# QuackenbushLab/phoenix

Hardware: AMD Instinct MI355X
Metric: ODE-RHS evals/sec (genes x trajectories) (higher is better)
Workload: dtype f32; 1 GPU; C4 breast_cancer ~11k-gene pseudotime, 256 trajectory intervals/GPU, dopri5 + adjoint; genes=11165, hidden=40, trajectories_per_gpu=256, method=dopri5, parallelism=trajectory-sharded x1, grouped gradient all-reduce, status_readback=deferred

## Files before the change

phoenix_amd/csrc/phx_adj3t.hip:

```cpp
#include <hip/hip_runtime.h>

#include <cstdlib>

#include "phx_solver.hpp"
#include "phx_host.hpp"

using namespace phxh;

#include "phx_mfma_common.inc"
#include "phx_mfma_v3common.inc"
#include "phx_mfma_adj3_tail.inc"

namespace phxh {

bool adj3_tail_on(const SolveArgs &a)
{
    const char *e = getenv("PHX_V3_TAIL");
    if (e && e[0] == '0') return false;
    const bool forced = e && e[0] == '1';
    return a.grads && a.d.HT == 3 && a.d.TG <= 256 && (forced || a.d.TG * a.d.ntg >= 4) &&
           (long long)tail_record_floats(a.d.Bt, a.d.ntg) <= a.PP;
}

bool launch_adj3_tail(const SolveArgs &a, const phx_grads *g, int overwrite, hipStream_t st)
{
    const D1 &d = a.d;
    hipLaunchKernelGGL((k3_tail_adj3<3>), dim3((unsigned int)(2 * d.nblk)), dim3(256), 0, st, d, a.w, a.net.g,
                       a.grad_y, a.adj_y0, a.PP, g->Ws, g->Wp, g->WaT, g->g, g->bs, g->bp, overwrite, g->Wa);
    return hipGetLastError() == hipSuccess;
}

}

extern "C" int phx_debug_adj3_tail_words(size_t *deferred, size_t *served)
{
    if (deferred) *deferred = (size_t)XH_DEFER * 4;
    if (served) *served = (size_t)XH_SERVED * 4;
    const char *e = getenv("PHX_V3_TAIL");
    return (e && e[0] == '0') ? 0 : 1;
}
```

phoenix_amd/csrc/phx_mfma_adj3_tail.inc:

```
namespace {

template <int HT>
__global__ __launch_bounds__(256, 2) void k3_tail_adj3(D1 d, W1 w, const float *__restrict__ gmul,
                                                       const float *__restrict__ grad_y, float *adj_y0, long long PP, float *gWs, float *gWp, float *gWaT,
                                                       float *gg, float *gbs, float *gbp, int overwrite, float *gWa)
{
    constexpr int F4 = 4 * HT, F2 = 2 * HT;
    __shared__ float4 red[4][F4][64];
    __shared__ __attribute__((aligned(16))) float ctl[4][16 * TR_N];
    __shared__ float dgred[4][16], bred[4][2][HT * 16];
    __shared__ int sdef[256];
    const int tid = threadIdx.x, lane = tid & 63, li = lane & 15, lq = lane >> 4;
    const int wv = __builtin_amdgcn_readfirstlane(tid >> 6);
    const int item = blockIdx.x, gb = item >> 1, s2 = item & 1;
    const int gtile = gb / d.NB, bl = gb % d.NB;
    const int N = d.N, H = d.H, B = d.B, Bt = d.Bt, ntg = d.ntg, TG = d.TG, G = d.G;
    const bool bias_item = item == 0;
    unsigned int *hdr = reinterpret_cast<unsigned int *>(w.cnt);
    for (int i = tid; i < 256; i += blockDim.x) sdef[i] = (i < TG && hdr[XH_DEFER + i] == 1u) ? 1 : 0;
    __syncthreads();

    const int tiles_wg = ntg * d.NB;
    const int lane32h = lane * 32 + 16 * s2, lane16 = lane * 16;
    const int gene0 = gb * 32;
    const long long og = (long long)d.nblk * (F4 * 2 * 256), obs = og + N, obp = obs + H;
    const __amdgpu_buffer_rsrc_t hrs = make_rsrc(w.hq, (unsigned int)((size_t)TG * ntg * 7 * F4 * 1024));
    auto ring = [&](int kb, int j) -> int { const int v = kb + j; return v >= 7 ? v - 7 : v; };
    float rr[4];
#pragma unroll
    for (int j = 0; j < 4; ++j) {
        const int gene = gene0 + gmap(lq, 4 * s2 + j);
        const float gm = gene < N ? gmul[gene] : 0.f;
        rr[j] = gm > 0.f ? gm : 0.f;
    }
    f32x4 gs_[HT], gp_[HT], ga_[F2];
    float dgacc[4], sbias[HT], pbias[HT];
#pragma unroll
    for (int f = 0; f < HT; ++f) { gs_[f] = (f32x4){0.f, 0.f, 0.f, 0.f}; gp_[f] = gs_[f]; sbias[f] = 0.f; pbias[f] = 0.f; }
#pragma unroll
    for (int f = 0; f < F2; ++f) ga_[f] = (f32x4){0.f, 0.f, 0.f, 0.f};
#pragma unroll
    for (int j = 0; j < 4; ++j) dgacc[j] = 0.f;

    for (int tt = wv; tt < TG * ntg; tt += 4) {
        const int grp = tt / ntg, ttl = tt % ntg;
        if (!sdef[grp]) continue;
        const float *blk = w.dtheta + (long long)grp * PP;
        __builtin_amdgcn_fence(__ATOMIC_SEQ_CST, "wavefront");
        reinterpret_cast<float4 *>(ctl[wv])[lane] = reinterpret_cast<const float4 *>(blk + (long long)ttl * 16 * TR_N)[lane];
        __builtin_amdgcn_fence(__ATOMIC_SEQ_CST, "wavefront");
        const int kb = __builtin_amdgcn_readfirstlane(reinterpret_cast<const int *>(blk + (long long)Bt * TR_N)[ttl]);
        const float *rec = ctl[wv] + li * TR_N;
        const int b = grp * Bt + ttl * 16 + li;
        const bool okb = b < B;
        const __amdgpu_buffer_rsrc_t trs = make_rsrc(w.scratch + (long long)(grp * G + gtile) * d.nvec * tiles_wg * 512,
                                                     (unsigned int)(d.nvec * tiles_wg * 2048));
        auto toff = [&](int v) -> int { return ((v * tiles_wg) + (ttl * d.NB + bl)) * 2048; };
        auto hoff = [&](int slot, int f) -> int { return (((grp * ntg + ttl) * 7 + slot) * F4 + f) * 1024; };
        float y0v[4], a0v[4], ky[7][4], ka[7][4];
        bload4(trs, lane32h, toff(C_Y0), y0v);
        bload4(trs, lane32h, toff(C_A0), a0v);
#pragma unroll
        for (int j = 0; j < 7; ++j) {
            bload4(trs, lane32h, toff(C_KY + ring(kb, j)), ky[j]);
            bload4(trs, lane32h, toff(C_KA + ring(kb, j)), ka[j]);
        }
        const float dts = rec[TR_DT], sg = rec[TR_SG];
        auto weighted = [&](int S) -> bool { return __any(rec[TR_W + S] != 0.f) != 0; };
        float h[F4][4];
        auto issue_h = [&](int S) {
            const int hs = ring(kb, S);
#pragma unroll
            for (int f = 0; f < F4; ++f) bload4(hrs, lane16, hoff(hs, (f + F2) % F4), h[f]);
        };
        if (weighted(0)) issue_h(0);
        float a1[4];
        auto stage = [&](auto Sc) {
            constexpr int S = decltype(Sc)::value;
            asm volatile("; PHXMARK tail stage %0" ::"n"(S));
            float ys[4], as[4];
            if (S == 0) {
#pragma unroll
                for (int j = 0; j < 4; ++j) { ys[j] = y0v[j]; as[j] = a0v[j]; }
            } else {
                float sy[4], sa[4];
#pragma unroll
                for (int j = 0; j < 4; ++j) { sy[j] = 0.f; sa[j] = 0.f; }
#pragma unroll
                for (int kk = 0; kk < S; ++kk) {
                    const float cf = DP_BETA[S > 0 ? S - 1 : 0][kk] * dts;
#pragma unroll
                    for (int j = 0; j < 4; ++j) { sy[j] += ky[kk][j] * cf; sa[j] += ka[kk][j] * cf; }
                }
#pragma unroll
                for (int j = 0; j < 4; ++j) { ys[j] = y0v[j] + sy[j]; as[j] = a0v[j] + sa[j]; }
            }
            if (S == 6) {
#pragma unroll
                for (int j = 0; j < 4; ++j) a1[j] = as[j];
            }
            if (weighted(S)) {
                const float wl = rec[TR_W + S];
                float w4[4];
#pragma unroll
                for (int r = 0; r < 4; ++r) w4[r] = ctl[wv][(4 * lq + r) * TR_N + TR_W + S];
                float an[4], ln[4], qn[4];
                act_pair_fast_pk<2>(ys, an, ln);
#pragma unroll
                for (int j = 0; j < 4; ++j) {
                    qn[j] = as[j] * rr[j];
                    dgacc[j] += wl * (as[j] * (-sg * ky[S][j]));
                }
                float at[4], lt[4], qt[4];
                xpose4(an, at, lane);
                xpose4(ln, lt, lane);
                xpose4(qn, qt, lane);
#pragma unroll
                for (int r = 0; r < 4; ++r) { at[r] *= w4[r]; lt[r] *= w4[r]; qt[r] *= w4[r]; }
#pragma unroll
                for (int f = 0; f < HT; ++f)
#pragma unroll
                    for (int r = 0; r < 4; ++r) {
                        gs_[f] = mfma4(h[f][r], at[r], gs_[f]);
                        gp_[f] = mfma4(h[HT + f][r], lt[r], gp_[f]);
                    }
#pragma unroll
                for (int f = 0; f < F2; ++f)
#pragma unroll
                    for (int r = 0; r < 4; ++r) ga_[f] = mfma4(h[F2 + f][r], qt[r], ga_[f]);
                if (bias_item) {
#pragma unroll
                    for (int f = 0; f < HT; ++f) {
                        sbias[f] += ((w4[0] * h[f][0] + w4[1] * h[f][1]) + w4[2] * h[f][2]) + w4[3] * h[f][3];
                        pbias[f] += ((w4[0] * h[HT + f][0] + w4[1] * h[HT + f][1]) + w4[2] * h[HT + f][2]) + w4[3] * h[HT + f][3];
                    }
                }
            }
            __builtin_amdgcn_sched_barrier(0);
            if (S < 6 && weighted(S < 6 ? S + 1 : 6)) issue_h(S + 1);
        };
        stage(I3<0>{}); stage(I3<1>{}); stage(I3<2>{}); stage(I3<3>{}); stage(I3<4>{}); stage(I3<5>{});
        const bool adv = rec[TR_ADV] != 0.f;
        float gy4[4];
        {
            const long long ro = (long long)b * N;
            const int g0 = gene0 + gmap(lq, 4 * s2);
            row_load4(grad_y, ro, g0, N, okb && adv, 0.f, gy4);
        }
        stage(I3<6>{});
        asm volatile("; PHXMARK tail accept");
        {
            float am[4];
#pragma unroll
            for (int j = 0; j < 4; ++j) am[j] = ka[0][j] * (dts * DP_CMID[0]);
#pragma unroll
            for (int kk = 2; kk < 6; ++kk) {
                const float cf = dts * DP_CMID[kk];
#pragma unroll
                for (int j = 0; j < 4; ++j) am[j] += ka[kk][j] * cf;
            }
            const InterpX ix = {rec[TR_X], rec[TR_X + 1], rec[TR_X + 2], rec[TR_X + 3]};
            float anew[4];
#pragma unroll
            for (int j = 0; j < 4; ++j) {
                am[j] += ka[6][j] * (dts * DP_CMID[6]);
                const float aout = interp_eval(a0v[j], a1[j], a0v[j] + am[j], ka[0][j], ka[6][j], dts, ix);
                anew[j] = adv ? aout + gy4[j] : a0v[j];
            }
            row_store4(adj_y0, (long long)b * N, gene0 + gmap(lq, 4 * s2), N, okb, anew);
        }
    }

#pragma unroll
    for (int f = 0; f < HT; ++f) {
        red[wv][0 * HT + f][lane] = make_float4(gs_[f][0], gs_[f][1], gs_[f][2], gs_[f][3]);
        red[wv][1 * HT + f][lane] = make_float4(gp_[f][0], gp_[f][1], gp_[f][2], gp_[f][3]);
        red[wv][2 * HT + f][lane] = make_float4(ga_[f][0], ga_[f][1], ga_[f][2], ga_[f][3]);
        red[wv][3 * HT + f][lane] = make_float4(ga_[HT + f][0], ga_[HT + f][1], ga_[HT + f][2], ga_[HT + f][3]);
    }
#pragma unroll
    for (int j = 0; j < 4; ++j) {
        float v = rr[j] > 0.f ? dgacc[j] * fast_rcp(rr[j]) : 0.f;
        v += __shfl_xor(v, 1, 64); v += __shfl_xor(v, 2, 64); v += __shfl_xor(v, 4, 64); v += __shfl_xor(v, 8, 64);
        if (li == 0) dgred[wv][lq * 4 + j] = v;
    }
    if (bias_item) {
#pragma unroll
        for (int f = 0; f < HT; ++f) {
            float sb = sbias[f], sp = pbias[f];
            sb += __shfl_xor(sb, 16, 64); sb += __shfl_xor(sb, 32, 64);
            sp += __shfl_xor(sp, 16, 64); sp += __shfl_xor(sp, 32, 64);
            if (lq == 0) { bred[wv][0][f * 16 + li] = sb; bred[wv][1][f * 16 + li] = sp; }
        }
    }
    __syncthreads();

    for (int mf = wv; mf < F4; mf += 4) {
        float4 sacc = red[0][mf][lane];
#pragma unroll
        for (int k = 1; k < 4; ++k) {
            const float4 v = red[k][mf][lane];
            sacc.x += v.x; sacc.y += v.y; sacc.z += v.z; sacc.w += v.w;
        }
        const long long slot = ((long long)gb * (F4 * 2) + mf * 2 + s2) * 64 + lane;
        for (int g = 0; g < TG; ++g)
            if (!sdef[g]) {
                const float4 v = reinterpret_cast<const float4 *>(w.dtheta + (long long)g * PP)[slot];
                sacc.x += v.x; sacc.y += v.y; sacc.z += v.z; sacc.w += v.w;
            }
        const int m = mf / HT, f = mf % HT;
        const int gene = gene0 + gmapC(li, s2);
        float *dst = (m == 0) ? gWs : (m == 1 ? gWp : (m == 2 ? gWaT : gWaT + (long long)H * N));
        const float o[4] = {sacc.x, sacc.y, sacc.z, sacc.w};
        if (gene >= N) continue;
        if (gWa && m >= 2) {
            float *q = gWa + (long long)gene * 2 * H + (m - 2) * H + 16 * f;
#pragma unroll
            for (int r = 0; r < 4; ++r) {
                const int rw = rho16(lq, r);
                if (16 * f + rw < H) q[rw] = overwrite ? o[r] : q[rw] + o[r];
            }
        } else {
#pragma unroll
            for (int r = 0; r < 4; ++r) {
                const int row = 16 * f + rho16(lq, r);
                if (row < H) {
                    float *q = dst + (long long)row * N + gene;
                    *q = overwrite ? o[r] : *q + o[r];
                }
            }
        }
    }
    if (tid < 16) {
        const int gene = gene0 + gmap(tid >> 2, 4 * s2 + (tid & 3));
        if (gene < N) {
            float v = ((dgred[0][tid] + dgred[1][tid]) + dgred[2][tid]) + dgred[3][tid];
            for (int g = 0; g < TG; ++g)
                if (!sdef[g]) v += w.dtheta[(long long)g * PP + og + gene];
            gg[gene] = overwrite ? v : gg[gene] + v;
        }
    }
    if (bias_item && tid >= 64 && tid < 64 + HT * 16) {
        const int e = tid - 64, f = e >> 4, i = e & 15;
        const int hid = 16 * f + rho16(i >> 2, i & 3);
        if (hid < H) {
            float sb = ((bred[0][0][e] + bred[1][0][e]) + bred[2][0][e]) + bred[3][0][e];
            float sp = ((bred[0][1][e] + bred[1][1][e]) + bred[2][1][e]) + bred[3][1][e];
            for (int g = 0; g < TG; ++g)
                if (!sdef[g]) { sb += w.dtheta[(long long)g * PP + obs + hid]; sp += w.dtheta[(long long)g * PP + obp + hid]; }
            gbs[hid] = overwrite ? sb : gbs[hid] + sb;
            gbp[hid] = overwrite ? sp : gbp[hid] + sp;
        }
    }
    if (bias_item && tid == 0) {
        int n = 0;
        for (int g = 0; g < TG; ++g) n += sdef[g];
        hdr[XH_SERVED] = (unsigned int)n;
    }
}

}
```

Baseline: 61.57 billion gene*trajectory RHS evals/s.

## Prefetch adjoint tail hidden rows into LDS across stages and tiles

Adds a default path (REGROWS=false) that streams the per-stage hidden-activation rows directly into LDS with buffer_load_lds and prefetches the next weighted stage, including the first weighted stage of the next served tile. Stage weight masks and ring offsets are peeked one tile ahead, and loads are interleaved with MFMAs through sched_group_barrier. It also makes FMA contraction explicit and moves the grad_y load into stage 5. The aim is to hide global-load latency of the h rows behind MFMA work, at the cost of hand-written waitcnt encodings and LDS reuse of the reduction buffer.

```diff
diff --git a/phoenix_amd/csrc/phx_adj3t.hip b/phoenix_amd/csrc/phx_adj3t.hip
--- a/phoenix_amd/csrc/phx_adj3t.hip
+++ b/phoenix_amd/csrc/phx_adj3t.hip
@@ -17,7 +17,7 @@
 {
     const char *e = getenv("PHX_V3_TAIL");
     if (e && e[0] == '0') return false;
-    const bool forced = e && e[0] == '1';
+    const bool forced = e && (e[0] == '1' || e[0] == '2');
     return a.grads && a.d.HT == 3 && a.d.TG <= 256 && (forced || a.d.TG * a.d.ntg >= 4) &&
            (long long)tail_record_floats(a.d.Bt, a.d.ntg) <= a.PP;
 }
@@ -25,7 +25,9 @@
 bool launch_adj3_tail(const SolveArgs &a, const phx_grads *g, int overwrite, hipStream_t st)
 {
     const D1 &d = a.d;
-    hipLaunchKernelGGL((k3_tail_adj3<3>), dim3((unsigned int)(2 * d.nblk)), dim3(256), 0, st, d, a.w, a.net.g,
+    const char *e = getenv("PHX_V3_TAIL");
+    auto kern = (e && e[0] == '2') ? k3_tail_adj3<3, true> : k3_tail_adj3<3, false>;
+    hipLaunchKernelGGL(kern, dim3((unsigned int)(2 * d.nblk)), dim3(256), 0, st, d, a.w, a.net.g,
                        a.grad_y, a.adj_y0, a.PP, g->Ws, g->Wp, g->WaT, g->g, g->bs, g->bp, overwrite, g->Wa);
     return hipGetLastError() == hipSuccess;
 }
diff --git a/phoenix_amd/csrc/phx_mfma_adj3_tail.inc b/phoenix_amd/csrc/phx_mfma_adj3_tail.inc
--- a/phoenix_amd/csrc/phx_mfma_adj3_tail.inc
+++ b/phoenix_amd/csrc/phx_mfma_adj3_tail.inc
@@ -1,10 +1,11 @@
 namespace {
 
-template <int HT>
+template <int HT, bool REGROWS>
 __global__ __launch_bounds__(256, 2) void k3_tail_adj3(D1 d, W1 w, const float *__restrict__ gmul,
                                                        const float *__restrict__ grad_y, float *adj_y0, long long PP, float *gWs, float *gWp, float *gWaT,
                                                        float *gg, float *gbs, float *gbp, int overwrite, float *gWa)
 {
+#pragma clang fp contract(off)
     constexpr int F4 = 4 * HT, F2 = 2 * HT;
     __shared__ float4 red[4][F4][64];
     __shared__ __attribute__((aligned(16))) float ctl[4][16 * TR_N];
@@ -42,21 +43,55 @@
 #pragma unroll
     for (int j = 0; j < 4; ++j) dgacc[j] = 0.f;
 
-    for (int tt = wv; tt < TG * ntg; tt += 4) {
+    const int T4 = TG * ntg;
+    auto next_served = [&](int tq) -> int {
+        do tq += 4; while (tq < T4 && __builtin_amdgcn_readfirstlane(sdef[tq / ntg]) == 0);
+        return tq;
+    };
+    auto peek_load = [&](int tq, float4 &wa, float4 &wb, int &kbq) {
+        const float *blk = w.dtheta + (long long)(tq / ntg) * PP;
+        const int tl = tq % ntg;
+        const float4 *r4 = reinterpret_cast<const float4 *>(blk + ((long long)tl * 16 + li) * TR_N + TR_W);
+        wa = r4[0]; wb = r4[1];
+        kbq = reinterpret_cast<const int *>(blk + (long long)Bt * TR_N)[tl];
+    };
+    auto peek_mask = [&](const float4 &wa, const float4 &wb) -> int {
+        const float ws[7] = {wa.x, wa.y, wa.z, wa.w, wb.x, wb.y, wb.z};
+        int m = 0;
+#pragma unroll
+        for (int S = 0; S < 7; ++S) m |= (__any(ws[S] != 0.f) != 0 ? 1 : 0) << S;
+        return __builtin_amdgcn_readfirstlane(m);
+    };
+    auto request = [&](int tq, int kbq, int S) {
+        const int base = ((tq * 7 + ring(kbq, S)) * F4) * 1024;
+#pragma unroll
+        for (int f = 0; f < F4; ++f)
+            __builtin_amdgcn_raw_ptr_buffer_load_lds(hrs, (__attribute__((address_space(3))) void *)&red[wv][f][0], 16,
+                                                     lane16, base + ((f + F2) % F4) * 1024, 0, 0);
+    };
+    int tt = next_served(wv - 4), kb = 0, mask = 0;
+    if (tt < T4) {
+        float4 wa, wb;
+        peek_load(tt, wa, wb, kb);
+        kb = __builtin_amdgcn_readfirstlane(kb);
+        mask = peek_mask(wa, wb);
+        if (!REGROWS && mask) request(tt, kb, __builtin_ctz(mask));
+    }
+    while (tt < T4) {
         const int grp = tt / ntg, ttl = tt % ntg;
-        if (!sdef[grp]) continue;
+        const int tn = next_served(tt);
+        float4 nwa, nwb;
+        int nkb;
+        peek_load(tn < T4 ? tn : tt, nwa, nwb, nkb);
         const float *blk = w.dtheta + (long long)grp * PP;
-        __builtin_amdgcn_fence(__ATOMIC_SEQ_CST, "wavefront");
-        reinterpret_cast<float4 *>(ctl[wv])[lane] = reinterpret_cast<const float4 *>(blk + (long long)ttl * 16 * TR_N)[lane];
-        __builtin_amdgcn_fence(__ATOMIC_SEQ_CST, "wavefront");
-        const int kb = __builtin_amdgcn_readfirstlane(reinterpret_cast<const int *>(blk + (long long)Bt * TR_N)[ttl]);
+        const float4 recs = reinterpret_cast<const float4 *>(blk + (long long)ttl * 16 * TR_N)[lane];
         const float *rec = ctl[wv] + li * TR_N;
         const int b = grp * Bt + ttl * 16 + li;
         const bool okb = b < B;
         const __amdgpu_buffer_rsrc_t trs = make_rsrc(w.scratch + (long long)(grp * G + gtile) * d.nvec * tiles_wg * 512,
                                                      (unsigned int)(d.nvec * tiles_wg * 2048));
         auto toff = [&](int v) -> int { return ((v * tiles_wg) + (ttl * d.NB + bl)) * 2048; };
-        auto hoff = [&](int slot, int f) -> int { return (((grp * ntg + ttl) * 7 + slot) * F4 + f) * 1024; };
+        auto hoff = [&](int slot, int f) -> int { return ((tt * 7 + slot) * F4 + f) * 1024; };
         float y0v[4], a0v[4], ky[7][4], ka[7][4];
         bload4(trs, lane32h, toff(C_Y0), y0v);
         bload4(trs, lane32h, toff(C_A0), a0v);
@@ -65,15 +100,23 @@
             bload4(trs, lane32h, toff(C_KY + ring(kb, j)), ky[j]);
             bload4(trs, lane32h, toff(C_KA + ring(kb, j)), ka[j]);
         }
+        __builtin_amdgcn_fence(__ATOMIC_SEQ_CST, "wavefront");
+        reinterpret_cast<float4 *>(ctl[wv])[lane] = recs;
+        __builtin_amdgcn_fence(__ATOMIC_SEQ_CST, "wavefront");
         const float dts = rec[TR_DT], sg = rec[TR_SG];
-        auto weighted = [&](int S) -> bool { return __any(rec[TR_W + S] != 0.f) != 0; };
+        const bool adv = rec[TR_ADV] != 0.f;
+        nkb = __builtin_amdgcn_readfirstlane(nkb);
+        const int nmask = tn < T4 ? peek_mask(nwa, nwb) : 0;
+        auto weighted = [&](int S) -> bool { return ((mask >> S) & 1) != 0; };
+        if (!REGROWS && mask == 0 && nmask) request(tn, nkb, __builtin_ctz(nmask));
         float h[F4][4];
         auto issue_h = [&](int S) {
             const int hs = ring(kb, S);
 #pragma unroll
             for (int f = 0; f < F4; ++f) bload4(hrs, lane16, hoff(hs, (f + F2) % F4), h[f]);
         };
-        if (weighted(0)) issue_h(0);
+        if (REGROWS && weighted(0)) issue_h(0);
+        float gy4[4];
         float a1[4];
         auto stage = [&](auto Sc) {
             constexpr int S = decltype(Sc)::value;
@@ -90,7 +133,7 @@
                 for (int kk = 0; kk < S; ++kk) {
                     const float cf = DP_BETA[S > 0 ? S - 1 : 0][kk] * dts;
 #pragma unroll
-                    for (int j = 0; j < 4; ++j) { sy[j] += ky[kk][j] * cf; sa[j] += ka[kk][j] * cf; }
+                    for (int j = 0; j < 4; ++j) { sy[j] = __builtin_fmaf(ky[kk][j], cf, sy[j]); sa[j] = __builtin_fmaf(ka[kk][j], cf, sa[j]); }
                 }
 #pragma unroll
                 for (int j = 0; j < 4; ++j) { ys[j] = y0v[j] + sy[j]; as[j] = a0v[j] + sa[j]; }
@@ -99,17 +142,42 @@
 #pragma unroll
                 for (int j = 0; j < 4; ++j) a1[j] = as[j];
             }
+            auto load_gy = [&]() {
+                const long long ro = (long long)b * N;
+                const int g0 = gene0 + gmap(lq, 4 * s2);
+                row_load4(grad_y, ro, g0, N, okb && adv, 0.f, gy4);
+            };
             if (weighted(S)) {
                 const float wl = rec[TR_W + S];
                 float w4[4];
+                int rbase = 0;
 #pragma unroll
                 for (int r = 0; r < 4; ++r) w4[r] = ctl[wv][(4 * lq + r) * TR_N + TR_W + S];
+                if (!REGROWS) {
+                    asm volatile("" ::: "memory");
+                    __builtin_amdgcn_s_waitcnt(0x0F70);
+                    asm volatile("" ::: "memory");
+#pragma unroll
+                    for (int f = 0; f < F4; ++f) {
+                        const float4 v = red[wv][f][lane];
+                        h[f][0] = v.x; h[f][1] = v.y; h[f][2] = v.z; h[f][3] = v.w;
+                    }
+                    asm volatile("" ::: "memory");
+                    __builtin_amdgcn_s_waitcnt(0xC07F);
+                    asm volatile("" ::: "memory");
+                    __builtin_amdgcn_sched_barrier(0);
+                    const int rest = mask >> (S + 1);
+                    const bool here = rest != 0, there = !here && nmask != 0;
+                    const int sq = here ? S + 1 + __builtin_ctz(rest | 64) : (there ? __builtin_ctz(nmask | 64) : S);
+                    rbase = (((there ? tn : tt) * 7 + ring(there ? nkb : kb, sq)) * F4) * 1024;
+                }
+                if (S == 5) load_gy();
                 float an[4], ln[4], qn[4];
                 act_pair_fast_pk<2>(ys, an, ln);
 #pragma unroll
                 for (int j = 0; j < 4; ++j) {
                     qn[j] = as[j] * rr[j];
-                    dgacc[j] += wl * (as[j] * (-sg * ky[S][j]));
+                    dgacc[j] = __builtin_fmaf(wl, as[j] * (-sg * ky[S][j]), dgacc[j]);
                 }
                 float at[4], lt[4], qt[4];
                 xpose4(an, at, lane);
@@ -117,6 +185,12 @@
                 xpose4(qn, qt, lane);
 #pragma unroll
                 for (int r = 0; r < 4; ++r) { at[r] *= w4[r]; lt[r] *= w4[r]; qt[r] *= w4[r]; }
+                if (!REGROWS) {
+#pragma unroll
+                    for (int f = 0; f < F4; ++f)
+                        __builtin_amdgcn_raw_ptr_buffer_load_lds(hrs, (__attribute__((address_space(3))) void *)&red[wv][f][0],
+                                                                 16, lane16, rbase + ((f + F2) % F4) * 1024, 0, 0);
+                }
 #pragma unroll
                 for (int f = 0; f < HT; ++f)
 #pragma unroll
@@ -128,26 +202,31 @@
                 for (int f = 0; f < F2; ++f)
 #pragma unroll
                     for (int r = 0; r < 4; ++r) ga_[f] = mfma4(h[F2 + f][r], qt[r], ga_[f]);
+                if (!REGROWS) {
+#pragma unroll
+                    for (int f = 0; f < F4; ++f) {
+                        __builtin_amdgcn_sched_group_barrier(0x008, 2, 0);
+                        __builtin_amdgcn_sched_group_barrier(0x010, 1, 0);
+                    }
+                }
                 if (bias_item) {
 #pragma unroll
                     for (int f = 0; f < HT; ++f) {
-                        sbias[f] += ((w4[0] * h[f][0] + w4[1] * h[f][1]) + w4[2] * h[f][2]) + w4[3] * h[f][3];
-                        pbias[f] += ((w4[0] * h[HT + f][0] + w4[1] * h[HT + f][1]) + w4[2] * h[HT + f][2]) + w4[3] * h[HT + f][3];
+                        float sb = __builtin_fmaf(w4[0], h[f][0], w4[1] * h[f][1]);
+                        float sp = __builtin_fmaf(w4[0], h[HT + f][0], w4[1] * h[HT + f][1]);
+                        sb = __builtin_fmaf(w4[3], h[f][3], __builtin_fmaf(w4[2], h[f][2], sb));
+                        sp = __builtin_fmaf(w4[3], h[HT + f][3], __builtin_fmaf(w4[2], h[HT + f][2], sp));
+                        sbias[f] += sb;
+                        pbias[f] += sp;
                     }
                 }
+            } else if (S == 5) {
+                load_gy();
             }
             __builtin_amdgcn_sched_barrier(0);
-            if (S < 6 && weighted(S < 6 ? S + 1 : 6)) issue_h(S + 1);
+            if (REGROWS && S < 6 && weighted(S < 6 ? S + 1 : 6)) issue_h(S + 1);
         };
-        stage(I3<0>{}); stage(I3<1>{}); stage(I3<2>{}); stage(I3<3>{}); stage(I3<4>{}); stage(I3<5>{});
-        const bool adv = rec[TR_ADV] != 0.f;
-        float gy4[4];
-        {
-            const long long ro = (long long)b * N;
-            const int g0 = gene0 + gmap(lq, 4 * s2);
-            row_load4(grad_y, ro, g0, N, okb && adv, 0.f, gy4);
-        }
-        stage(I3<6>{});
+        stage(I3<0>{}); stage(I3<1>{}); stage(I3<2>{}); stage(I3<3>{}); stage(I3<4>{}); stage(I3<5>{}); stage(I3<6>{});
         asm volatile("; PHXMARK tail accept");
         {
             float am[4];
@@ -157,20 +236,22 @@
             for (int kk = 2; kk < 6; ++kk) {
                 const float cf = dts * DP_CMID[kk];
 #pragma unroll
-                for (int j = 0; j < 4; ++j) am[j] += ka[kk][j] * cf;
+                for (int j = 0; j < 4; ++j) am[j] = __builtin_fmaf(ka[kk][j], cf, am[j]);
             }
             const InterpX ix = {rec[TR_X], rec[TR_X + 1], rec[TR_X + 2], rec[TR_X + 3]};
             float anew[4];
 #pragma unroll
             for (int j = 0; j < 4; ++j) {
-                am[j] += ka[6][j] * (dts * DP_CMID[6]);
+                am[j] = __builtin_fmaf(ka[6][j], dts * DP_CMID[6], am[j]);
                 const float aout = interp_eval(a0v[j], a1[j], a0v[j] + am[j], ka[0][j], ka[6][j], dts, ix);
                 anew[j] = adv ? aout + gy4[j] : a0v[j];
             }
             row_store4(adj_y0, (long long)b * N, gene0 + gmap(lq, 4 * s2), N, okb, anew);
         }
-    }
-
+        tt = tn; kb = nkb; mask = nmask;
+    }
+
+    if (!REGROWS) __builtin_amdgcn_s_waitcnt(0x0F70);
 #pragma unroll
     for (int f = 0; f < HT; ++f) {
         red[wv][0 * HT + f][lane] = make_float4(gs_[f][0], gs_[f][1], gs_[f][2], gs_[f][3]);
```

Result: no change. 62.05 billion gene*trajectory RHS evals/s (median of 6 runs) (+0.8%).
